# lambdaclass/simpleworks

Hardware: AMD Instinct MI355X
Metric: Marlin prove() constraints/sec at 2^20 R1CS; G1 MSM points/sec (higher is better)
Workload: dtype u32 limbs (384-bit Montgomery Fq for G1, 256-bit Fr); 1 GPU; marlin_prove: synthetic R1CS, 2^20 constraints = variables = non-zeros per matrix (|H| = |K| = 2^20), SRS + proving key device resident; per_gpu_units=1048576, multi_gpu=replicas (one proof per rank)

## Files before the change

simpleworks_amd/_lib.py:

```python
import ctypes
import json
import os

import numpy as np

_HERE = os.path.dirname(os.path.abspath(__file__))
LIB_PATH = os.environ.get("SWM_LIB_PATH") or os.path.join(_HERE, "libswmarlin.so")

_u64p = ctypes.POINTER(ctypes.c_uint64)
_u32p = ctypes.POINTER(ctypes.c_uint32)
_vp = ctypes.c_void_p
_sz = ctypes.c_size_t
_int = ctypes.c_int

ABI = {
    "swm_version": (_int, []),
    "swm_strerror": (ctypes.c_char_p, [_int]),
    "swm_init": (_int, [_int, ctypes.POINTER(_vp)]),
    "swm_destroy": (None, [_vp]),
    "swm_last_error": (ctypes.c_char_p, [_vp]),
    "swm_set_stream": (_int, [_vp, _vp]),
    "swm_set_msm_sharding": (_int, [_vp, ctypes.c_uint, ctypes.c_uint, _vp, _vp]),
    "swm_rccl_unique_id": (_int, [ctypes.c_void_p]),
    "swm_rccl_init": (_int, [_vp, ctypes.c_void_p, ctypes.c_uint, ctypes.c_uint]),
# ... 1225 lines not shown
        self._poly(3, buf, buf.shape[0], 0, z_mont, pc, out)
        return out

    def selftest_ntt_from(self, src_mont, log_n, inverse=False, coset=False):
        src = np.ascontiguousarray(src_mont, dtype=np.uint64).reshape(-1, 4).copy()
        out = np.zeros((1 << log_n, 4), dtype=np.uint64)
        self._poly(4 + int(bool(inverse)) + 2 * int(bool(coset)), src, src.shape[0], log_n, None, None, out)
        return out, src

    def selftest_ntt_cosets(self, coeffs_mont, log_n, ks):
        src = np.ascontiguousarray(coeffs_mont, dtype=np.uint64).reshape(-1, 4).copy()
        kk = np.ascontiguousarray(ks, dtype=np.uint64).reshape(-1)
        out = np.zeros((kk.size << log_n, 4), dtype=np.uint64)
        self._check(self.lib.swm_selftest_poly(self.h, 9, src.ctypes.data, src.shape[0], log_n, _p64(np.zeros(4, np.uint64)),
                                               _p64(kk), kk.size, out.ctypes.data), "swm_selftest_poly")
        return out.reshape(kk.size, 1 << log_n, 4)

    def selftest_intt_cosets3(self, evals_mont, log_n):
        ev = np.ascontiguousarray(evals_mont, dtype=np.uint64).reshape(-1, 4).copy()
        out = np.zeros_like(ev)
        self._poly(10, ev, ev.shape[0], log_n, None, None, out)
        return out

    def selftest_scan(self, words):
        w = np.ascontiguousarray(words, dtype=np.uint32).reshape(-1)
        out = np.zeros(w.size + 1, dtype=np.uint32)
        self._poly(8, w, w.size, 0, None, None, out)
        return out[:-1], int(out[-1])

    def selftest_spmv_plan(self, rowptr, col, val_mont, z_mont):
        rowptr = np.ascontiguousarray(rowptr, dtype=np.uint32)
        col = np.ascontiguousarray(col, dtype=np.uint32)
        val = np.ascontiguousarray(val_mont, dtype=np.uint64).reshape(-1, 4)
        z = np.ascontiguousarray(z_mont, dtype=np.uint64).reshape(-1, 4)
        rows = rowptr.shape[0] - 1
        out = np.zeros((rows, 4), dtype=np.uint64)
        counts = np.zeros(2, dtype=np.uint32)
        self._check(self.lib.swm_selftest_spmv_plan(self.h, _p32(rowptr), _p32(col) if col.size else None,
                                                    _p64(val) if val.size else None, rows, _p64(z), z.shape[0], _p64(out),
                                                    _p32(counts)), "swm_selftest_spmv_plan")
        return out, int(counts[0]), int(counts[1])

    MSM_ROLES = {None: 0, "none": 0, "lead": 1, "follow": 2}
    MSM_DEFER = {"off": 0, "on": 1, "prover": 2}

    def selftest_msm_jobs(self, sets, vectors, jobs, montgomery=False, defer_tail="prover", pipe_min=0):
# ... 23 lines not shown
```

simpleworks_amd/csrc/devops.cuh:

```cuda
#pragma once
#include <chrono>
#include <exception>
#include <functional>
#include <utility>
#include <atomic>
#include "context.h"
#include "ff.cuh"
#include "fill.cuh"
#include "fr29.cuh"
#include "host/chacha.h"
#include "host/marlin_types.h"

namespace swm {

int ntt_run(swm_ctx* ctx, void* d_data, unsigned log_n, int inverse, int coset);
int ntt_run_from(swm_ctx* ctx, void* d_data, unsigned log_n, int inverse, int coset, const void* first_src, size_t src_len);
int ntt_cosets_fwd(swm_ctx* ctx, const void* coeffs, size_t len, unsigned log_n, const unsigned* ks, unsigned ncos, void* out);
int ntt_cosets_inv(swm_ctx* ctx, void* data, unsigned log_n, unsigned ncos);
int ntt_sharded_run(swm_ctx* ctx, void* d_local, unsigned log_n, int inverse, int blocks_in);
struct SpmvPlanHost {
    uint64_t nnz = 0, max_row = 0;
    std::vector<uint32_t> chunks, lrows;
};
struct SpmvPlan {
    uint64_t nnz = 0, max_row = 0;
    const uint32_t* d_chunks = nullptr;
    const uint32_t* d_lrows = nullptr;
    uint32_t n_chunks = 0, n_lrows = 0;
};
void spmv_plan_build(const uint32_t* rowptr, size_t rows, SpmvPlanHost* plan);
int spmv_run(swm_ctx* ctx, const void* d_rowptr, const void* d_col, const void* d_val, const void* d_z, void* d_out,
             size_t rows, const SpmvPlan* plan = nullptr);
int batch_inverse_run(swm_ctx* ctx, void* d, size_t n);

inline void hip_check(swm_ctx* ctx, hipError_t e, const char* what) {
    if (e != hipSuccess) {
        set_err(ctx, SWM_ERR_HIP, "%s: %s", what, hipGetErrorString(e));
        throw MarlinError(e == hipErrorOutOfMemory ? SWM_ERR_OOM : SWM_ERR_HIP, std::string(what) + ": " + hipGetErrorString(e));
    }
}
inline void rc_check(swm_ctx* ctx, int rc) {
    if (rc != SWM_OK) throw MarlinError(rc, ctx->err);
}

template <class T>
struct DBuf {
    swm_ctx* ctx = nullptr;
    T* p = nullptr;
    size_t n = 0, cap = 0;
    DBuf() {}
    DBuf(swm_ctx* c, size_t count) : ctx(c), n(count) {
        void* q = nullptr;
        rc_check(c, pool_alloc(c, (count ? count : 1) * sizeof(T), &q, &cap));
        p = (T*)q;
    }
    DBuf(const DBuf&) = delete;
// ... 824 lines not shown
```

simpleworks_amd/csrc/fr29.cuh:

```cuda
#pragma once
#include "ff.cuh"

namespace swm {

struct Fr29 {
    uint32_t l[9];
};
static constexpr uint32_t M29 = (1u << 29) - 1;
struct Fr29Consts {
    static constexpr uint32_t P[9] = SWM_FR29_P;
    static constexpr uint32_t ONE[9] = SWM_FR29_ONE;
    static constexpr uint32_t P2[9] = SWM_FR29_2P;
};

__device__ __forceinline__ Fr29 fr29_unpack(const Fr& a) {
    Fr29 r;
#pragma unroll
    for (int i = 0; i < 9; i++) {
        const int bit = 29 * i, w = bit >> 5, off = bit & 31;
        uint32_t v = a.v[w] >> off;
        if (off > 3 && w + 1 < 8) v |= a.v[w + 1] << (32 - off);
        r.l[i] = i < 8 ? (v & M29) : v;
    }
    return r;
// ... 17 lines not shown
    return r;
}
__device__ __forceinline__ Fr29 fr29_normalize(const Fr29& a) {
    Fr29 r;
    uint32_t c = 0;
#pragma unroll
    for (int i = 0; i < 8; i++) {
        uint32_t t = a.l[i] + c;
        r.l[i] = t & M29;
        c = t >> 29;
    }
    r.l[8] = a.l[8] + c;
    return r;
}
__device__ __forceinline__ Fr29 fr29_add(const Fr29& a, const Fr29& b) {
    Fr29 r;
#pragma unroll
    for (int i = 0; i < 9; i++) r.l[i] = a.l[i] + b.l[i];
    return r;
}
struct Spread29 {
    uint32_t l[9];
};
__device__ __forceinline__ Fr29 fr29_sub(const Fr29& a, const Fr29& b, const Spread29& sp) {
    Fr29 r;
#pragma unroll
    for (int i = 0; i < 9; i++) r.l[i] = a.l[i] + sp.l[i] - b.l[i];
    return r;
}
__device__ __forceinline__ Fr29 fr29_mul(const Fr29& a, const Fr29& b) {
    Fr29 r;
    uint32_t m[9];
    uint64_t acc = 0;
#pragma unroll
    for (int k = 0; k < 9; k++) {
#pragma unroll
        for (int i = 0; i <= k; i++) acc += (uint64_t)a.l[i] * b.l[k - i];
#pragma unroll
        for (int i = 0; i < k; i++) acc += (uint64_t)m[i] * Fr29Consts::P[k - i];
        m[k] = (0u - (uint32_t)acc) & M29;
        acc = (acc + m[k]) >> 29;
    }
#pragma unroll
    for (int k = 9; k < 17; k++) {
#pragma unroll
        for (int i = k - 8; i < 9; i++) acc += (uint64_t)a.l[i] * b.l[k - i];
// ... 44 lines not shown
```

simpleworks_amd/csrc/marlin.hip:

```cpp
#include <stdlib.h>
#include <string.h>
#include <algorithm>
#include <chrono>
#include <functional>
#include <memory>
#include <type_traits>
#include "devops.cuh"
#include "g1.cuh"
#include "host/ahp.h"

#include "msm.h"
using namespace swm;

#define LAUNCHX(ctx, name, kernel, grid, block, shmem, ...)                         \
    do {                                                                            \
        prof_begin(ctx, name);                                                      \
        hipLaunchKernelGGL(kernel, grid, block, shmem, (ctx)->stream, __VA_ARGS__); \
        prof_end(ctx);                                                              \
        hip_check(ctx, hipGetLastError(), name);                                    \
    } while (0)

#include "host/pk_codec.h"
#include "host/host_handles.h"
struct swm_srs {
    ~swm_srs() {
        if (d_powers) (void)hipFree(d_powers);
    }
    size_t max_degree = 0;
    bool in_subgroup = false;
    G1Affine* d_powers = nullptr;
    std::vector<G1Affine> gamma_powers;
    G2Affine h, beta_h;
};

namespace {

struct DevCsr {
    DBuf<uint32_t> rowptr, col;
    DVec val;
    size_t rows = 0, nnz = 0;
    DBuf<uint32_t> plan_chunks, plan_lrows;
    SpmvPlan plan;
};
struct MatrixArith {
    DVec row, col, val, row_col;
    DVec row_K, col_K, val_K;
    DVec row_B, col_B, val_B, row_col_B;
};
struct GammaTable {
    std::vector<G1Affine> t;
    const G1Affine& at(int j, int w, int d) const { return t[((size_t)j * 64 + w) * 15 + (d - 1)]; }
};

}

struct swm_pk {
    ~swm_pk() {
        if (d_powers) (void)hipFree(d_powers);
        if (d_powers28) (void)hipFree(d_powers28);
        if (d_shifted) (void)hipFree(d_shifted);
        if (d_shifted28) (void)hipFree(d_shifted28);
        if (d_powers_te) (void)hipFree(d_powers_te);
        if (d_shifted_te) (void)hipFree(d_shifted_te);
    }
    int device = 0;
    std::atomic<int> refs{1};
    void own_blocks() {
        for (DevCsr* m : {&a, &b, &c, &at, &bt, &ct}) {
            m->rowptr.detach(); m->col.detach(); m->val.detach(); m->plan_chunks.detach(); m->plan_lrows.detach();
        }
        for (MatrixArith& m : ar)
            for (DVec* v : {&m.row, &m.col, &m.val, &m.row_col, &m.row_K, &m.col_K, &m.val_K, &m.row_B, &m.col_B, &m.val_B, &m.row_col_B})
                v->detach();
    }
    IndexInfo info;
    uint64_t H = 0, K = 0, X = 0, B = 0;
    unsigned logH = 0, logK = 0, logX = 0, logB = 0;
    HostCsr ha, hb, hc;
    DevCsr a, b, c, at, bt, ct;
    MatrixArith ar[3];
    G1Affine* d_powers = nullptr;
    G1Affine* d_powers28 = nullptr;
    G1Affine* d_shifted = nullptr;
    G1Affine* d_shifted28 = nullptr;
    size_t n_powers = 0, n_shifted = 0, shift_base = 0;
    size_t srs_max_degree = 0;
    unsigned tab_c = 0, shtab_c = 0;
    G1TE* d_powers_te = nullptr;
    G1TE* d_shifted_te = nullptr;
    bool in_powers(size_t offset, size_t n) const { return offset + n <= n_powers; }
    void bases_at(size_t offset, size_t n, const G1Affine** b, const G1Affine** b28, MsmTable* tab) const {
        *tab = MsmTable();
        if (in_powers(offset, n)) {
            *b = d_powers + offset;
            *b28 = d_powers28 + offset;
            if (tab_c) *tab = MsmTable{d_powers_te ? nullptr : d_powers28, n_powers, tab_c, offset, d_powers_te};
// ... 617 lines not shown

__device__ __forceinline__ uint64_t reindex_by_subdomain(uint64_t H, uint64_t X, uint64_t index) {
    uint64_t period = H / X;
    if (index < X) return index * period;
    uint64_t i = index - X, x = period - 1;
    return i + (i / x) + 1;
}

void arithmetize(swm_ctx* ctx, swm_pk& pk, const HostCsr& m, MatrixArith& ar) {
    const uint64_t K = pk.K, H = pk.H, X = pk.X;
    std::vector<uint32_t> rows(m.nnz());
    for (size_t r = 0; r < m.rows(); r++)
        for (uint32_t k = m.rowptr[r]; k < m.rowptr[r + 1]; k++) rows[k] = (uint32_t)r;
    DBuf<uint32_t> d_rows(ctx, std::max<size_t>(m.nnz(), 1)), d_cols(ctx, std::max<size_t>(m.nnz(), 1));
    DVec d_vals(ctx, std::max<size_t>(m.nnz(), 1));
    if (m.nnz()) {
        d_rows.upload(rows.data(), m.nnz());
        d_cols.upload(m.col.data(), m.nnz());
        d_vals.upload(m.val.data(), m.nnz());
    }
    ar.row_K = DVec(ctx, K);
    ar.col_K = DVec(ctx, K);
    ar.val_K = DVec(ctx, K);
    DVec rc_K(ctx, K);
    PowTable wt = root_pow_table(ctx, pk.logH);
    Fr h_inv = HDomain(H).size_inv;
    size_t nnz = m.nnz();
    Fr *prow = ar.row_K.p, *pcol = ar.col_K.p, *pval = ar.val_K.p, *prc = rc_K.p;
    const uint32_t *drows = d_rows.p, *dcols = d_cols.p;
    const Fr* dvals = d_vals.p;
    ew(ctx, "index_arith", K, [=] __device__(size_t k) {
        Fr rv, cv, vv;
        if (k < nnz) {
            rv = wt.at(reindex_by_subdomain(H, X, dcols[k]));
            cv = wt.at(drows[k]);
            vv = fp_mul(fp_mul(dvals[k], rv), h_inv);
        } else {
            rv = fp_one<Fr>();
            cv = fp_one<Fr>();
            vv = fp_zero<Fr>();
        }
        prow[k] = rv;
        pcol[k] = cv;
        pval[k] = vv;
        prc[k] = fp_mul(rv, cv);
    });
    auto interp = [&](const DVec& evals) {
        return dv_ntt_from(ctx, evals.p, K, pk.logK, true);
    };
    ar.row = interp(ar.row_K);
    ar.col = interp(ar.col_K);
    ar.val = interp(ar.val_K);
    ar.row_col = interp(rc_K);
    auto on_b = [&](const DVec& coeffs) {
        return dv_ntt_from(ctx, coeffs.p, K, pk.logB, false);
    };
    ar.row_B = on_b(ar.row);
    ar.col_B = on_b(ar.col);
    ar.val_B = on_b(ar.val);
    ar.row_col_B = on_b(ar.row_col);
}

void install_committer_key(swm_ctx* ctx, swm_pk& pk, const G1Affine* powers, size_t n_powers, const G1Affine* shifted,
                           size_t n_shifted, bool device_src, bool in_subgroup) {
// ... 204 lines not shown
        poly[H] = fp_add(poly[H], rho);
    });
}
void div_vh(swm_ctx* ctx, const Fr* q, size_t part, size_t total, Fr* h, Fr* g) {
    ew(ctx, "div_vh", 3 * part, [=] __device__(size_t j) {
        Fr acc = q[j + part];
        if (j + 2 * part < total) acc = fp_add(acc, q[j + 2 * part]);
        if (j + 3 * part < total) acc = fp_add(acc, q[j + 3 * part]);
        h[j] = acc;
        if (j < part) g[j] = fp_add(q[j], acc);
    });
}
void div_vk(swm_ctx* ctx, const Fr* q, size_t part, size_t total, Fr* h) {
    ew(ctx, "div_vk", 3 * part, [=] __device__(size_t j) {
        Fr acc = fp_zero<Fr>();
        for (uint64_t i = 1; j + i * part < total; i++) acc = fp_add(acc, q[j + i * part]);
        h[j] = acc;
    });
}
#ifndef SWM_OUTER_COSETS
#define SWM_OUTER_COSETS 1
#endif
static constexpr uint64_t OUTER_COSETS_MIN_H = 16;
struct Cosets3 {
    Fr p0, p1, p2;
};
__device__ __forceinline__ Cosets3 cosets3_solve(const Fr& u0, const Fr& u1, const Fr& u2, const Fr& iota, const Fr& half) {
    const Fr p1 = fp_mul(fp_sub(u0, u2), half);
    const Fr e = fp_mul(fp_add(u0, u2), half);
    const Fr d = fp_sub(u1, fp_mul(iota, p1));
    return {fp_mul(fp_add(e, d), half), p1, fp_mul(fp_sub(e, d), half)};
}
static Fr fr_half() { return fp_inv(fp_from_u64<Fr>(2)); }
struct RAlphaNumerators {
    Fr n0, n1, n2, n3;
    __device__ __forceinline__ Fr at(size_t i) const {
        const unsigned q = (unsigned)(i & 3);
        return q == 0 ? n0 : q == 1 ? n1 : q == 2 ? n2 : n3;
    }
};
RAlphaNumerators r_alpha_numerators(const Fr& alpha, unsigned logH, uint64_t M) {
    Fr aH = alpha;
    for (unsigned i = 0; i < logH; i++) aH = fp_sqr(aH);
    Fr i4 = HDomain(M).gen;
    for (unsigned i = 0; i < logH; i++) i4 = fp_sqr(i4);
    return {fp_sub(aH, fp_one<Fr>()), fp_sub(aH, i4), fp_sub(aH, fp_sqr(i4)), fp_sub(aH, fp_mul(fp_sqr(i4), i4))};
// ... 19 lines not shown
__device__ __forceinline__ Fr round2_outer_form(const Fr& eta_a, const Fr& eta_b, const Fr& eta_c, const Fr& ra, const Fr& a,
                                                const Fr& b, const Fr& z, const Fr& t) {
    const Fr summed = fp_add(fp_add(fp_mul(eta_c, fp_mul(a, b)), fp_mul(eta_a, a)), fp_mul(eta_b, b));
    return fp_sub(fp_mul(ra, summed), fp_mul(z, t));
}
struct IndexOnB {
    const Fr *ar, *ac, *arc, *av;
    const Fr *br, *bc, *brc, *bv;
    const Fr *cr, *cc, *crc, *cv;
};
struct Round3Challenges {
    Fr alpha, beta, ab, eta_a, eta_b, eta_c, vhab;
};
__device__ __forceinline__ Fr round3_a_minus_bf(const IndexOnB& x, const Round3Challenges& c, size_t i, const Fr& f) {
    Fr da = fp_add(fp_sub(fp_sub(c.ab, fp_mul(x.ar[i], c.alpha)), fp_mul(c.beta, x.ac[i])), x.arc[i]);
    Fr db = fp_add(fp_sub(fp_sub(c.ab, fp_mul(x.br[i], c.alpha)), fp_mul(c.beta, x.bc[i])), x.brc[i]);
    Fr dc = fp_add(fp_sub(fp_sub(c.ab, fp_mul(x.cr[i], c.alpha)), fp_mul(c.beta, x.cc[i])), x.crc[i]);
    Fr dbc = fp_mul(db, dc);
    Fr t = fp_add(fp_add(fp_mul(fp_mul(c.eta_a, x.av[i]), dbc), fp_mul(fp_mul(fp_mul(c.eta_b, x.bv[i]), da), dc)),
                  fp_mul(fp_mul(fp_mul(c.eta_c, x.cv[i]), da), db));
    Fr a_val = fp_mul(c.vhab, t);
    Fr b_val = fp_mul(da, dbc);
    return fp_sub(a_val, fp_mul(b_val, f));
}
struct ProveState {
    ChaChaRng& zk;
    PhaseTrace& tr;
    const ProveShape shape;
    const ShardPlan sp;
    const uint64_t H, K, X, Bsz, M;
    const unsigned logM;
    const size_t nvars, ninst;
    const size_t mask_len;
    const HDomain dh;
    const std::vector<Fr> public_input;
    FiatShamirRng fs;
    VerifierState st;
    Fr rho_w, rho_a, rho_b;
    int lane = 0;
    LPoly P_w, P_za, P_zb, P_mask, P_t, P_g1, P_h1, P_g2, P_h2;
    LPoly idx_polys[12];
    std::map<std::string, LPoly*> polys;
    CommitJob j1[4], j2[3], j3[2];
    std::vector<Commitment> comms1 = std::vector<Commitment>(4), comms2 = std::vector<Commitment>(3),
                            comms3 = std::vector<Commitment>(2);
    bool mask_late = false;
// ... 209 lines not shown
        out[i] = v;
    });
    s.e_z = on_round2_layout(ctx, s, z_poly.p, H + 1);
}

void round1_commitments(swm_ctx* ctx, const swm_pk& pk, ProveState& s) {
    pc_commit_blind(pk, &s.j1[0], &s.zk, &s.P_w.rand);
    pc_commit_blind(pk, &s.j1[1], &s.zk, &s.P_za.rand);
    pc_commit_blind(pk, &s.j1[2], &s.zk, &s.P_zb.rand);
    pc_commit_blind(pk, &s.j1[3], nullptr, &s.P_mask.rand);
    if (s.mask_pieces > 1) {
        Fr c0 = s.mask.download(0, 1)[0];
        Fr c0s = fp_to_std(c0);
        G1XYZZ extra = g1_mul_limbs(pk.vk.vk.g, c0s.v, 8);
        for (unsigned k = 0; k + 1 < s.mask_pieces; k++) g1_add(extra, commit_wait(ctx, &s.mask_part[k]));
        s.j1[3].has_extra = true;
        s.j1[3].extra = extra;
    }
    commit_gather(ctx, {&s.j1[0].plain, &s.j1[1].plain, &s.j1[2].plain, &s.j1[3].plain});
    pc_commit_end_round(ctx, pk, {&s.j1[0], &s.j1[1], &s.j1[2], &s.j1[3]}, {&s.zk, &s.zk, &s.zk, nullptr},
                        {&s.P_w.rand, &s.P_za.rand, &s.P_zb.rand, &s.P_mask.rand}, s.comms1.data());
}

void r_alpha_on_h(swm_ctx* ctx, const swm_pk& pk, ProveState& s) {
    const Fr alpha = s.st.alpha;
    PowTable wh = root_pow_table(ctx, pk.logH);
    Fr* rh = s.r_alpha_evals.p;
    ew(ctx, "r_alpha_den", s.H, [=] __device__(size_t i) { rh[i] = fp_sub(alpha, wh.at(i)); });
    rc_check(ctx, batch_inverse_run(ctx, rh, s.H));
    Fr vh = s.dh.vanishing(alpha);
    ew(ctx, "r_alpha_scale", s.H, [=] __device__(size_t i) { rh[i] = fp_mul(rh[i], vh); });
}
void r_alpha(swm_ctx* ctx, const swm_pk& pk, ProveState& s) {
    const Fr alpha = s.st.alpha;
    s.r_alpha_evals = DVec(ctx, s.H);
    {
        Fr a4h = alpha;
        for (unsigned i = 0; i < s.logM; i++) a4h = fp_sqr(a4h);
        s.ra_closed_form = !fp_is_one(a4h) && !sw(SW_RALPHA_TRANSFORMS);
    }
    if (!s.ra_closed_form) return r_alpha_on_h(ctx, pk, s);
    const size_t n = s.cosets ? 3 * s.H : s.sp.Mloc;
    s.e_ra = DVec(ctx, n);
    PowTable wt = root_pow_table(ctx, s.logM);
    Fr* out = s.e_ra.p;
    Fr* rh = s.r_alpha_evals.p;
    const RAlphaNumerators nu = r_alpha_numerators(alpha, pk.logH, s.M);
    with_product_map(s.sp, s.sp.r2, n, s.cosets, pk.logH, [&](auto map) {
        ew(ctx, "r_alpha_den", n, [=] __device__(size_t p) { out[p] = fp_sub(alpha, wt.at(map.index(p))); });
        rc_check(ctx, batch_inverse_run(ctx, out, n));
        ew(ctx, "r_alpha_scale", n, [=] __device__(size_t p) {
            const size_t i = map.index(p);
            const Fr v = fp_mul(out[p], nu.at(i));
            out[p] = v;
            if constexpr (!std::is_same_v<decltype(map), BlocksMap>)
                if ((i & 3) == 0) rh[i >> 2] = v;
        });
    });
// ... 28 lines not shown
                if (k % ratio != 0) {
                    const size_t wi = k - k / ratio - 1;
                    zk = wi < nwit ? zz[ninst + wi] : fp_zero<Fr>();
                }
                q[k] = round2_outer_form(eta_a, eta_b, eta_c, rh[k], za[k], zb[k], zk, th[k]);
            });
        }
        dv_ntt(ctx, s.t_poly, pk.logH, true);
    }
    s.tr.tick("r2: t polynomial enqueued");
    s.P_t.p = s.t_poly.p;
    s.P_t.n = H;
    pc_commit_begin(ctx, pk, &s.lane, s.P_t.p, s.P_t.n, false, 0, false, &s.j2[0]);
}

void round2_q1(swm_ctx* ctx, const swm_pk& pk, ProveState& s) {
    const uint64_t H = s.H, M = s.M;
    const size_t Mloc = s.sp.Mloc;
    const Fr eta_a = s.st.eta_a, eta_b = s.st.eta_b, eta_c = s.st.eta_c;
    const size_t off = s.cosets ? H : 0, n = s.cosets ? 2 * H : Mloc;
    if (!s.cosets) s.q1 = DVec(ctx, Mloc);
    const Fr* mp = s.mask.p;
    {
        const Fr* pra = s.e_ra.p + off;
        if (!s.ra_closed_form) {
            DVec ra_poly = dv_ntt_from(ctx, s.r_alpha_evals.p, H, pk.logH, true);
            s.e_ra = on_round2_layout(ctx, s, ra_poly.p, H);
            pra = s.e_ra.p;
        }
        DVec e_t = on_round2_layout(ctx, s, s.t_poly.p, H);
        Fr* out = s.q1.p + off;
        const Fr *pza = s.e_za.p, *pzb = s.e_zb.p, *pt = e_t.p, *pz = s.e_z.p;
        ew(ctx, "round2_pointwise", n, [=] __device__(size_t i) {
            out[i] = round2_outer_form(eta_a, eta_b, eta_c, pra[i], pza[i], pzb[i], pz[i], pt[i]);
        });
        s.e_za.release();
        s.e_zb.release();
        s.e_z.release();
    }
    s.h1 = DVec(ctx, 3 * H);
    s.g1x = DVec(ctx, H);
    Fr* q = s.q1.p;
    if (s.cosets) {
        rc_check(ctx, ntt_cosets_inv(ctx, q, pk.logH, 3));
        Fr *h = s.h1.p, *g = s.g1x.p;
        const Fr iota = HDomain(4).gen, half = fr_half();
        ew(ctx, "q1_cosets_solve_div_vh", H, [=] __device__(size_t j) {
            const Cosets3 c = cosets3_solve(q[j], q[j + H], q[j + 2 * H], iota, half);
            const Fr p0 = fp_add(c.p0, mp[j]), p1 = fp_add(c.p1, mp[j + H]), p2 = fp_add(c.p2, mp[j + 2 * H]);
            const Fr hj = fp_add(p1, p2);
            h[j] = hj;
// ... 35 lines not shown
    pc_commit_begin(ctx, pk, &s.lane, s.P_h1.p, s.P_h1.n, false, 0, false, &s.j2[2]);
    pc_commit_begin(ctx, pk, &s.lane, s.P_g1.p, s.P_g1.n, true, H - 2, true, &s.j2[1]);
    commit_flush(ctx);
    Fr rem0 = s.g1x.download(0, 1)[0];
    bool unsat = !fp_is_zero(rem0);
    pc_commit_blind(pk, &s.j2[0], nullptr, &s.P_t.rand);
    pc_commit_blind(pk, &s.j2[1], &s.zk, &s.P_g1.rand);
    pc_commit_blind(pk, &s.j2[2], nullptr, &s.P_h1.rand);
    commit_gather(ctx, {&s.j2[0].plain, &s.j2[1].plain, &s.j2[1].shifted, &s.j2[2].plain});
    pc_commit_end_round(ctx, pk, {&s.j2[0], &s.j2[1], &s.j2[2]}, {nullptr, &s.zk, nullptr},
                        {&s.P_t.rand, &s.P_g1.rand, &s.P_h1.rand}, s.comms2.data());
    if (unsat && !ctx->emulated_exchange)
        throw MarlinError(SWM_ERR_UNSATISFIED, "outer sumcheck does not hold: constraint system is not satisfied");
}

void round3_polys(swm_ctx* ctx, const swm_pk& pk, ProveState& s) {
    const uint64_t K = s.K, Bsz = s.Bsz;
    const Fr alpha = s.st.alpha, beta = s.st.beta;
    const Fr eta_a = s.st.eta_a, eta_b = s.st.eta_b, eta_c = s.st.eta_c;
    const Fr vhab = fp_mul(s.dh.vanishing(alpha), s.dh.vanishing(beta));
    s.f = DVec(ctx, K);
    const bool f_cosets = SWM_OUTER_COSETS && !s.sp.r3 && Bsz == 4 * K && K >= OUTER_COSETS_MIN_H;
    DVec f_K;
    {
        DVec inv(ctx, 3 * K);
        for (int m = 0; m < 3; m++) {
            Fr* out = inv.p + (size_t)m * K;
            const Fr *rk = pk.ar[m].row_K.p, *ck = pk.ar[m].col_K.p;
            ew(ctx, "round3_den_K", K, [=] __device__(size_t i) { out[i] = fp_mul(fp_sub(beta, rk[i]), fp_sub(alpha, ck[i])); });
        }
        rc_check(ctx, batch_inverse_run(ctx, inv.p, 3 * K));
        Fr* out = s.f.p;
        const Fr *ia = inv.p, *ib = inv.p + K, *ic = inv.p + 2 * K;
        const Fr *va = pk.ar[0].val_K.p, *vb = pk.ar[1].val_K.p, *vc = pk.ar[2].val_K.p;
        if (f_cosets) {
            f_K = DVec(ctx, K);
            out = f_K.p;
        }
        ew(ctx, "round3_f_K", K, [=] __device__(size_t i) {
            Fr t = fp_add(fp_add(fp_mul(fp_mul(eta_a, va[i]), ia[i]), fp_mul(fp_mul(eta_b, vb[i]), ib[i])),
                          fp_mul(fp_mul(eta_c, vc[i]), ic[i]));
            out[i] = fp_mul(vhab, t);
        });
        if (f_cosets) rc_check(ctx, ntt_run_from(ctx, s.f.p, pk.logK, 1, 0, f_K.p, K));
        else dv_ntt(ctx, s.f, pk.logK, true);
    }
    s.P_g2.p = s.f.p + 1; s.P_g2.n = K - 1; s.P_g2.has_bound = true; s.P_g2.bound = K - 2;
// ... 838 lines not shown
}
int swm_pk_deserialize(swm_ctx* ctx, const uint8_t* bytes, size_t len, swm_pk** out) {
    return swm_pk_deserialize_ex(ctx, bytes, len, 0, out);
}
int swm_r1cs_is_satisfied(swm_ctx* ctx, const swm_r1cs* cs, int* ok, size_t* first_bad) {
    if (!ctx || !cs || !ok) return SWM_ERR_INVALID_ARG;
    SWM_ON_DEVICE(ctx);
    SWM_GUARD(ctx, is_satisfied_impl(ctx, cs, ok, first_bad));
}

static void selftest_poly_impl(swm_ctx* ctx, int op, void* data, size_t n, size_t m, const uint64_t* z, const uint64_t* pieces,
                               size_t npieces, void* out) {
    Fr zz = fp_zero<Fr>();
    if (z) memcpy(zz.v, z, 32);
    if (op == 8) {
        DBuf<uint32_t> in(ctx, n), res(ctx, n);
        if (n) in.upload((const uint32_t*)data, n);
        const uint32_t total = scan_exclusive_u32(ctx, in.p, res.p, n);
        std::vector<uint32_t> h = res.download(0, n);
        if (n) memcpy(out, h.data(), n * 4);
        ((uint32_t*)out)[n] = total;
        return;
    }
    DVec a(ctx, n);
    if (n) a.upload((const Fr*)data, n);
    if (op == 9) {
        unsigned ks[4];
        for (size_t c = 0; c < npieces; c++) ks[c] = (unsigned)pieces[c];
        DVec t(ctx, npieces << m);
        rc_check(ctx, ntt_cosets_fwd(ctx, a.p, n, (unsigned)m, ks, (unsigned)npieces, t.p));
        std::vector<Fr> h = t.download(0, t.n);
        memcpy(out, h.data(), t.n * sizeof(Fr));
        return;
    }
    if (op == 10) {
        const size_t N = (size_t)1 << m;
        rc_check(ctx, ntt_cosets_inv(ctx, a.p, (unsigned)m, 3));
        DVec t(ctx, 3 * N);
        const Fr* u = a.p;
        Fr* o = t.p;
        const Fr iota = HDomain(4).gen, half = fr_half();
        ew(ctx, "cosets3_solve", N, [=] __device__(size_t j) {
            const Cosets3 c = cosets3_solve(u[j], u[j + N], u[j + 2 * N], iota, half);
            o[j] = c.p0;
            o[j + N] = c.p1;
            o[j + 2 * N] = c.p2;
// ... 13 lines not shown
    } else if (op == 2) {
        const Fr v = poly_eval(ctx, a.p, n, zz);
        memcpy(out, v.v, sizeof(Fr));
    } else if (op == 3) {
        for (size_t i = 0; i < npieces; i++)
            if (pieces[2 * i] > n || pieces[2 * i + 1] > n - pieces[2 * i]) throw MarlinError(SWM_ERR_INVALID_ARG, "piece out of range");
        DVec res(ctx, npieces);
        std::vector<EvalItem> items;
        for (size_t i = 0; i < npieces; i++) items.push_back({a.p + pieces[2 * i], (size_t)pieces[2 * i + 1], res.p + i});
        EvalPoint ep = eval_point(ctx, zz);
        poly_eval_many(ctx, items, ep);
        std::vector<Fr> h = res.download(0, npieces);
        if (npieces) memcpy(out, h.data(), npieces * sizeof(Fr));
    } else {
        DVec t = dv_ntt_from(ctx, a.p, n, (unsigned)m, ((op - 4) & 1) != 0, ((op - 4) & 2) != 0);
        std::vector<Fr> h = t.download(0, t.n);
        memcpy(out, h.data(), t.n * sizeof(Fr));
        std::vector<Fr> s = a.download(0, n);
        if (n) memcpy(data, s.data(), n * sizeof(Fr));
    }
}
int swm_selftest_poly(swm_ctx* ctx, int op, void* data, size_t n, size_t m, const uint64_t z[4], const uint64_t* pieces,
                      size_t npieces, void* out) {
    if (!ctx || op < 0 || op > 10 || (n && !data)) return SWM_ERR_INVALID_ARG;
    if ((op >= 1 && op <= 3 && !z) || (op == 0 && (!z || m == 0)) || (op != 0 && !out) || (op == 3 && npieces && !pieces))
        return SWM_ERR_INVALID_ARG;
    if (op >= 4 && op <= 7 && (m < 1 || m > 28 || n > ((size_t)1 << m))) return SWM_ERR_INVALID_ARG;
    if (op == 9) {
        if (m < 1 || m > 26 || n > ((size_t)2 << m) || npieces < 1 || npieces > 4 || !pieces) return SWM_ERR_INVALID_ARG;
        for (size_t c = 0; c < npieces; c++)
            if (pieces[c] > 3) return SWM_ERR_INVALID_ARG;
    }
    if (op == 10 && (m < 1 || m > 26 || n != ((size_t)3 << m))) return SWM_ERR_INVALID_ARG;
    SWM_ON_DEVICE(ctx);
    SWM_GUARD(ctx, selftest_poly_impl(ctx, op, data, n, m, z, pieces, npieces, out));
}
static void selftest_spmv_plan_impl(swm_ctx* ctx, const uint32_t* rowptr, const uint32_t* col, const uint64_t* val, size_t rows,
                                    const uint64_t* z, size_t z_len, uint64_t* out, uint32_t* plan_counts) {
    const size_t nnz = rowptr[rows];
    HostCsr m;
    m.rowptr.assign(rowptr, rowptr + rows + 1);
    m.col.assign(col, col + nnz);
    m.val.resize(nnz);
    if (nnz) memcpy(m.val.data(), val, nnz * sizeof(Fr));
    DevCsr d = upload_csr(ctx, m);
    DVec dz(ctx, z_len), o(ctx, rows);
    dz.upload((const Fr*)z, z_len);
// ... 103 lines not shown
```

simpleworks_amd/csrc/ntt.hip:

```cpp
#include <atomic>
#include "context.h"
#include "ff.cuh"
#include "fr29.cuh"
#include <string.h>
#include <algorithm>
#include <vector>

namespace swm {

static constexpr int NTT_THREADS = 256;
static constexpr unsigned NTT_MAX_LOG_R = 10;

struct NttPassArgs {
    const Fr* src;
    Fr* dst;
    unsigned log_n, log_r, log_ns;
    const Fr* tw_small;
    const Fr* tw_lo;
    const Fr* tw_hi;
    const Fr* cs_lo;
    const Fr* cs_hi;
    uint64_t src_len;
    const Fr* pass_tw;
    int coset_in;
// ... 354 lines not shown
    static const bool off = sw(SW_NTT_PASS_TABLES) == 0;
    if (off) return SWM_OK;
    const uint64_t key = (1ull << 51) | ((uint64_t)log_n << 20) | ((uint64_t)log_ns << 10) | ((uint64_t)log_r << 1) | (inverse ? 1 : 0);
    auto it = ctx->ntt_small.find(key);
    if (it == ctx->ntt_small.end()) {
        const size_t count = (size_t)1 << (log_ns + log_r);
        if (ctx->ntt_pass_table_bytes + count * sizeof(Fr) > ((size_t)4 << 30)) return SWM_OK;
        void* d = nullptr;
        if (hipMalloc(&d, count * sizeof(Fr)) != hipSuccess) {
            (void)hipGetLastError();
            return SWM_OK;
        }
        hipLaunchKernelGGL(ntt_build_pass_tw, dim3((unsigned)((count + 255) / 256)), dim3(256), 0, ctx->stream,
                           reinterpret_cast<const Fr*>(rt29->lo), reinterpret_cast<const Fr*>(rt29->hi), log_ns, log_r,
                           log_n - log_ns - log_r, reinterpret_cast<Fr*>(d));
        SWM_HIP(ctx, hipGetLastError());
        ctx->ntt_pass_table_bytes += count * sizeof(Fr);
        it = ctx->ntt_small.emplace(key, d).first;
    }
    *out = reinterpret_cast<const Fr*>(it->second);
    return SWM_OK;
}

static Spread29 lazy_spread(unsigned k, unsigned borrows) {
    Spread29 sp;
    uint64_t carry = 0;
    for (int i = 0; i < 9; i++) {
        uint64_t t = (uint64_t)Fr29Consts::P[i] * k + carry;
        sp.l[i] = i < 8 ? (uint32_t)(t & M29) : (uint32_t)t;
        carry = t >> 29;
    }
    sp.l[0] += borrows << 29;
    for (int i = 1; i < 8; i++) sp.l[i] += (borrows << 29) - borrows;
    sp.l[8] -= borrows;
    return sp;
}
static LazyPlan lazy_plan(unsigned log_r, unsigned b_in) {
    LazyPlan P;
    memset(&P, 0, sizeof(P));
    unsigned B = b_in;
    P.r2 = lazy_spread(2 * B, 1);
    if (log_r & 1) B = std::max(2 * B, 2u);
    const unsigned nsteps = log_r / 2;
    for (unsigned st = 0; st < nsteps && st < 6; st++) {
        P.s1[st] = lazy_spread(2 * B, 1);
        P.s2[st] = lazy_spread(4 * B, 2);
        const bool red = 4 * B > 64 || st + 1 == nsteps;
        if (red) P.reduce |= 1u << st;
        B = red ? 4 : 4 * B;
    }
    P.s4 = lazy_spread(4, 1);
    P.out_below_2r = B <= 2 ? 1u : 0u;
    return P;
}

int ntt_run_from(swm_ctx* ctx, void* d_data, unsigned log_n, int inverse, int coset, const void* first_src, size_t src_len);
int ntt_run(swm_ctx* ctx, void* d_data, unsigned log_n, int inverse, int coset) {
    return ntt_run_from(ctx, d_data, log_n, inverse, coset, nullptr, 0);
}
// ... 220 lines not shown
```

simpleworks_amd/csrc/vec.hip:

```cpp
#include <string.h>
#include "context.h"
#include "fq28.cuh"
#include "fr29.cuh"
#include "frinv.cuh"
#include "g1.cuh"

namespace swm {

__global__ void __launch_bounds__(256) vec_mul_kernel(const Fr* __restrict__ a, const Fr* __restrict__ b,
                                                      Fr* __restrict__ out, size_t n) {
    SWM_LIGHT_KERNEL();
    for (size_t i = blockIdx.x * (size_t)blockDim.x + threadIdx.x; i < n; i += (size_t)gridDim.x * blockDim.x)
        out[i] = fp_mul(a[i], b[i]);
}

static constexpr int BINV_CHUNK = 16, BINV_CHUNK_SMALL = 4;
static constexpr int BINV_THREADS = 256;
template <int BINV_CHUNK>
__global__ void __launch_bounds__(BINV_THREADS) batch_inverse_kernel29(Fr* __restrict__ v, size_t n) {
    SWM_LIGHT_KERNEL();
    __shared__ Fr sp[BINV_THREADS], ss[BINV_THREADS];
    __shared__ Fr s_inv;
    const unsigned tid = threadIdx.x;
    size_t t = blockIdx.x * (size_t)blockDim.x + tid;
// ... 37 lines not shown
            }
        }
    }
}

int vec_mul_run(swm_ctx* ctx, const void* a, const void* b, void* out, size_t n) {
    if (n == 0) return SWM_OK;
    unsigned grid = (unsigned)std::min<size_t>((n + 255) / 256, 256 * 32);
    SWM_LAUNCH(ctx, "vec_mul", vec_mul_kernel, dim3(grid), dim3(256), 0, (const Fr*)a, (const Fr*)b, (Fr*)out, n);
    return SWM_OK;
}
int batch_inverse_run(swm_ctx* ctx, void* d, size_t n) {
    if (n == 0) return SWM_OK;
    static constexpr size_t small_below = 262144;
    if (n <= small_below) {
        const size_t threads = (n + BINV_CHUNK_SMALL - 1) / BINV_CHUNK_SMALL;
        const dim3 grid((unsigned)((threads + BINV_THREADS - 1) / BINV_THREADS));
        SWM_LAUNCH(ctx, "batch_inverse", batch_inverse_kernel29<BINV_CHUNK_SMALL>, grid, dim3(BINV_THREADS), 0, (Fr*)d, n);
        return SWM_OK;
    }
    const size_t threads = (n + BINV_CHUNK - 1) / BINV_CHUNK;
    const dim3 grid((unsigned)((threads + BINV_THREADS - 1) / BINV_THREADS));
    SWM_LAUNCH(ctx, "batch_inverse", batch_inverse_kernel29<BINV_CHUNK>, grid, dim3(BINV_THREADS), 0, (Fr*)d, n);
    return SWM_OK;
}

template <class F>
__global__ void __launch_bounds__(256) selftest_mul_kernel(const F* a, const F* b, F* out, size_t n) {
    size_t i = blockIdx.x * (size_t)blockDim.x + threadIdx.x;
    if (i < n) out[i] = fp_mul(a[i], b[i]);
}
template <class F>
__global__ void __launch_bounds__(256) selftest_mul_chain(F* out, int iters) {
    size_t i = blockIdx.x * (size_t)blockDim.x + threadIdx.x;
    F a = fp_one<F>(), b = fp_one<F>();
    a.v[0] ^= (uint32_t)i;
    b.v[1] ^= (uint32_t)(i * 2654435761u);
    for (int k = 0; k < iters; k++) {
        a = fp_mul(a, b);
        b = fp_mul(b, a);
    }
    out[i] = fp_add(a, b);
}
__global__ void __launch_bounds__(256) selftest_mul28_kernel(const Fq* a, const Fq* b, Fq* out, size_t n) {
    size_t i = blockIdx.x * (size_t)blockDim.x + threadIdx.x;
    if (i < n) out[i] = fq28_pack(fq28_canonical(fq28_mul(fq28_unpack(a[i]), fq28_unpack(b[i]))));
// ... 160 lines not shown
```

Before: 22.74 million constraints/s.

## Compute Lagrange-kernel evaluations via product tower and gather-based round-3 f

Replaces the batch-inverse computation of r(alpha, X) on H (and on the round-2 cosets) with a multiplicative product-tower kernel that builds the evaluations from squared powers of the challenge. Round 3 no longer inverts per-matrix denominators over K. Instead it evaluates r(beta, .) on H with the same tower and gathers r_beta[row] * r_alpha[col] using new uint32 index arrays stored in the proving key. This trades batch inversions and some NTT work for random-access gathers and extra key memory, and adds selftests for the new kernels.

Result: no change. 22.90 million constraints/s (median of 6 runs) (+0.7%).

```diff
diff --git a/simpleworks_amd/_lib.py b/simpleworks_amd/_lib.py
--- a/simpleworks_amd/_lib.py
+++ b/simpleworks_amd/_lib.py
@@ -1271,6 +1271,39 @@
         self._poly(10, ev, ev.shape[0], log_n, None, None, out)
         return out
 
+    R_TOWER_LAYOUTS = {"pieces": 0, "dense": 1, "h": 2}
+
+    def selftest_r_tower(self, c_mont, log_n, cosets, layout="pieces"):
+        kk = np.ascontiguousarray(cosets, dtype=np.uint64).reshape(-1)
+        n = 1 << log_n
+        rows = {"pieces": kk.size * n, "dense": 4 * n, "h": n}[layout]
+        out = np.zeros((rows, 4), dtype=np.uint64)
+        zz = np.ascontiguousarray(c_mont, dtype=np.uint64).reshape(4)
+        self._check(self.lib.swm_selftest_poly(self.h, 11, None, self.R_TOWER_LAYOUTS[layout], log_n, _p64(zz), _p64(kk), kk.size,
+                                               out.ctypes.data), "swm_selftest_poly")
+        return out.reshape(kk.size, n, 4) if layout == "pieces" else out
+
+    def selftest_round3_f(self, r_beta_mont, r_alpha_mont, vals_mont, idx, etas_mont):
+        rb = np.ascontiguousarray(r_beta_mont, dtype=np.uint64).reshape(-1, 4)
+        ra = np.ascontiguousarray(r_alpha_mont, dtype=np.uint64).reshape(-1, 4)
+        ix = np.ascontiguousarray(idx, dtype=np.uint32)
+        K = ix.shape[-1]
+        va = np.ascontiguousarray(vals_mont, dtype=np.uint64).reshape(3 * K, 4)
+        assert ra.shape == rb.shape and ix.shape == (3, 2, K)
+        data = np.ascontiguousarray(np.concatenate([rb, ra, va, np.asarray(etas_mont, dtype=np.uint64).reshape(3, 4)]))
+        words = np.zeros((6 * K + 1) // 2, dtype=np.uint64)
+        words.view(np.uint32)[:6 * K] = ix.reshape(-1)
+        out = np.zeros((K, 4), dtype=np.uint64)
+        self._check(self.lib.swm_selftest_poly(self.h, 12, data.ctypes.data, rb.shape[0], K, _p64(np.zeros(4, np.uint64)),
+                                               _p64(words), words.size, out.ctypes.data), "swm_selftest_poly")
+        return out
+
+    def selftest_pk_index_arrays(self, pk_handle, K):
+        out = np.zeros((3, 2, K), dtype=np.uint32)
+        self._check(self.lib.swm_selftest_poly(self.h, 13, pk_handle, K, 0, _p64(np.zeros(4, np.uint64)), None, 0,
+                                               out.ctypes.data), "swm_selftest_poly")
+        return out
+
     def selftest_scan(self, words):
         w = np.ascontiguousarray(words, dtype=np.uint32).reshape(-1)
         out = np.zeros(w.size + 1, dtype=np.uint32)
diff --git a/simpleworks_amd/csrc/devops.cuh b/simpleworks_amd/csrc/devops.cuh
--- a/simpleworks_amd/csrc/devops.cuh
+++ b/simpleworks_amd/csrc/devops.cuh
@@ -32,6 +32,7 @@
 int spmv_run(swm_ctx* ctx, const void* d_rowptr, const void* d_col, const void* d_val, const void* d_z, void* d_out,
              size_t rows, const SpmvPlan* plan = nullptr);
 int batch_inverse_run(swm_ctx* ctx, void* d, size_t n);
+int r_tower_run(swm_ctx* ctx, const void* c, unsigned m, const unsigned* cosets, unsigned ncos, int dense, void* out);
 
 inline void hip_check(swm_ctx* ctx, hipError_t e, const char* what) {
     if (e != hipSuccess) {
diff --git a/simpleworks_amd/csrc/fr29.cuh b/simpleworks_amd/csrc/fr29.cuh
--- a/simpleworks_amd/csrc/fr29.cuh
+++ b/simpleworks_amd/csrc/fr29.cuh
@@ -63,6 +63,19 @@
 struct Spread29 {
     uint32_t l[9];
 };
+inline Spread29 lazy_spread(unsigned k, unsigned borrows) {
+    Spread29 sp;
+    uint64_t carry = 0;
+    for (int i = 0; i < 9; i++) {
+        uint64_t t = (uint64_t)Fr29Consts::P[i] * k + carry;
+        sp.l[i] = i < 8 ? (uint32_t)(t & M29) : (uint32_t)t;
+        carry = t >> 29;
+    }
+    sp.l[0] += borrows << 29;
+    for (int i = 1; i < 8; i++) sp.l[i] += (borrows << 29) - borrows;
+    sp.l[8] -= borrows;
+    return sp;
+}
 __device__ __forceinline__ Fr29 fr29_sub(const Fr29& a, const Fr29& b, const Spread29& sp) {
     Fr29 r;
 #pragma unroll
diff --git a/simpleworks_amd/csrc/marlin.hip b/simpleworks_amd/csrc/marlin.hip
--- a/simpleworks_amd/csrc/marlin.hip
+++ b/simpleworks_amd/csrc/marlin.hip
@@ -46,6 +46,7 @@
     DVec row, col, val, row_col;
     DVec row_K, col_K, val_K;
     DVec row_B, col_B, val_B, row_col_B;
+    DBuf<uint32_t> row_idx, col_idx;
 };
 struct GammaTable {
     std::vector<G1Affine> t;
@@ -72,6 +73,10 @@
         for (MatrixArith& m : ar)
             for (DVec* v : {&m.row, &m.col, &m.val, &m.row_col, &m.row_K, &m.col_K, &m.val_K, &m.row_B, &m.col_B, &m.val_B, &m.row_col_B})
                 v->detach();
+        for (MatrixArith& m : ar) {
+            m.row_idx.detach();
+            m.col_idx.detach();
+        }
     }
     IndexInfo info;
     uint64_t H = 0, K = 0, X = 0, B = 0;
@@ -735,6 +740,8 @@
     ar.row_K = DVec(ctx, K);
     ar.col_K = DVec(ctx, K);
     ar.val_K = DVec(ctx, K);
+    ar.row_idx = DBuf<uint32_t>(ctx, K);
+    ar.col_idx = DBuf<uint32_t>(ctx, K);
     DVec rc_K(ctx, K);
     PowTable wt = root_pow_table(ctx, pk.logH);
     Fr h_inv = HDomain(H).size_inv;
@@ -742,17 +749,23 @@
     Fr *prow = ar.row_K.p, *pcol = ar.col_K.p, *pval = ar.val_K.p, *prc = rc_K.p;
     const uint32_t *drows = d_rows.p, *dcols = d_cols.p;
     const Fr* dvals = d_vals.p;
+    uint32_t *pri = ar.row_idx.p, *pci = ar.col_idx.p;
     ew(ctx, "index_arith", K, [=] __device__(size_t k) {
         Fr rv, cv, vv;
+        uint32_t ri = 0, ci = 0;
         if (k < nnz) {
-            rv = wt.at(reindex_by_subdomain(H, X, dcols[k]));
-            cv = wt.at(drows[k]);
+            ri = (uint32_t)reindex_by_subdomain(H, X, dcols[k]);
+            ci = drows[k];
+            rv = wt.at(ri);
+            cv = wt.at(ci);
             vv = fp_mul(fp_mul(dvals[k], rv), h_inv);
         } else {
             rv = fp_one<Fr>();
             cv = fp_one<Fr>();
             vv = fp_zero<Fr>();
         }
+        pri[k] = ri;
+        pci[k] = ci;
         prow[k] = rv;
         pcol[k] = cv;
         pval[k] = vv;
@@ -1003,6 +1016,9 @@
 #define SWM_OUTER_COSETS 1
 #endif
 static constexpr uint64_t OUTER_COSETS_MIN_H = 16;
+#ifndef SWM_PRELUDE_PRODUCTS
+#define SWM_PRELUDE_PRODUCTS 1
+#endif
 struct Cosets3 {
     Fr p0, p1, p2;
 };
@@ -1068,6 +1084,21 @@
     Fr a_val = fp_mul(c.vhab, t);
     Fr b_val = fp_mul(da, dbc);
     return fp_sub(a_val, fp_mul(b_val, f));
+}
+struct Round3Tables {
+    Fr eta[3];
+    const Fr* val[3];
+    const uint32_t *row_idx[3], *col_idx[3];
+};
+void round3_f_on_k(swm_ctx* ctx, const Fr* r_beta, const Fr* r_alpha, const Round3Tables& tables, size_t K, Fr* out) {
+    const Round3Tables x = tables;
+    ew(ctx, "round3_f_K", K, [=] __device__(size_t k) {
+        Fr acc = fp_zero<Fr>();
+#pragma unroll
+        for (int m = 0; m < 3; m++)
+            acc = fp_add(acc, fp_mul(fp_mul(x.eta[m], x.val[m][k]), fp_mul(r_beta[x.row_idx[m][k]], r_alpha[x.col_idx[m][k]])));
+        out[k] = acc;
+    });
 }
 struct ProveState {
     ChaChaRng& zk;
@@ -1323,18 +1354,33 @@
                         {&s.P_w.rand, &s.P_za.rand, &s.P_zb.rand, &s.P_mask.rand}, s.comms1.data());
 }
 
+void r_on_h(swm_ctx* ctx, const swm_pk& pk, const Fr& c, Fr* out) {
+    static const unsigned h_alone[1] = {0};
+    rc_check(ctx, r_tower_run(ctx, &c, pk.logH, h_alone, 1, 0, out));
+}
 void r_alpha_on_h(swm_ctx* ctx, const swm_pk& pk, ProveState& s) {
     const Fr alpha = s.st.alpha;
+    Fr* rh = s.r_alpha_evals.p;
+    if (SWM_PRELUDE_PRODUCTS) return r_on_h(ctx, pk, alpha, rh);
     PowTable wh = root_pow_table(ctx, pk.logH);
-    Fr* rh = s.r_alpha_evals.p;
     ew(ctx, "r_alpha_den", s.H, [=] __device__(size_t i) { rh[i] = fp_sub(alpha, wh.at(i)); });
     rc_check(ctx, batch_inverse_run(ctx, rh, s.H));
     Fr vh = s.dh.vanishing(alpha);
     ew(ctx, "r_alpha_scale", s.H, [=] __device__(size_t i) { rh[i] = fp_mul(rh[i], vh); });
 }
+void r_alpha_rest(swm_ctx* ctx, const swm_pk& pk, ProveState& s) {
+    static const unsigned rest[2] = {1, 2}, all[4] = {0, 1, 2, 3};
+    s.e_ra = DVec(ctx, s.cosets ? 2 * s.H : s.M);
+    if (s.cosets) rc_check(ctx, r_tower_run(ctx, &s.st.alpha, pk.logH, rest, 2, 0, s.e_ra.p));
+    else rc_check(ctx, r_tower_run(ctx, &s.st.alpha, pk.logH, all, 4, 1, s.e_ra.p));
+}
 void r_alpha(swm_ctx* ctx, const swm_pk& pk, ProveState& s) {
     const Fr alpha = s.st.alpha;
     s.r_alpha_evals = DVec(ctx, s.H);
+    if (SWM_PRELUDE_PRODUCTS && !s.sp.r2) {
+        s.ra_closed_form = !sw(SW_RALPHA_TRANSFORMS);
+        return r_alpha_on_h(ctx, pk, s);
+    }
     {
         Fr a4h = alpha;
         for (unsigned i = 0; i < s.logM; i++) a4h = fp_sqr(a4h);
@@ -1409,11 +1455,16 @@
     if (!s.cosets) s.q1 = DVec(ctx, Mloc);
     const Fr* mp = s.mask.p;
     {
-        const Fr* pra = s.e_ra.p + off;
+        const Fr* pra;
         if (!s.ra_closed_form) {
             DVec ra_poly = dv_ntt_from(ctx, s.r_alpha_evals.p, H, pk.logH, true);
             s.e_ra = on_round2_layout(ctx, s, ra_poly.p, H);
             pra = s.e_ra.p;
+        } else if (SWM_PRELUDE_PRODUCTS && !s.sp.r2) {
+            r_alpha_rest(ctx, pk, s);
+            pra = s.e_ra.p;
+        } else {
+            pra = s.e_ra.p + off;
         }
         DVec e_t = on_round2_layout(ctx, s, s.t_poly.p, H);
         Fr* out = s.q1.p + off;
@@ -1495,7 +1546,24 @@
     s.f = DVec(ctx, K);
     const bool f_cosets = SWM_OUTER_COSETS && !s.sp.r3 && Bsz == 4 * K && K >= OUTER_COSETS_MIN_H;
     DVec f_K;
-    {
+    if (SWM_PRELUDE_PRODUCTS) {
+        DVec r_beta(ctx, s.H);
+        r_on_h(ctx, pk, beta, r_beta.p);
+        Fr* out = s.f.p;
+        if (f_cosets) {
+            f_K = DVec(ctx, K);
+            out = f_K.p;
+        }
+        Round3Tables t{{eta_a, eta_b, eta_c}, {}, {}, {}};
+        for (int m = 0; m < 3; m++) {
+            t.val[m] = pk.ar[m].val_K.p;
+            t.row_idx[m] = pk.ar[m].row_idx.p;
+            t.col_idx[m] = pk.ar[m].col_idx.p;
+        }
+        round3_f_on_k(ctx, r_beta.p, s.r_alpha_evals.p, t, K, out);
+        if (f_cosets) rc_check(ctx, ntt_run_from(ctx, s.f.p, pk.logK, 1, 0, f_K.p, K));
+        else dv_ntt(ctx, s.f, pk.logK, true);
+    } else {
         DVec inv(ctx, 3 * K);
         for (int m = 0; m < 3; m++) {
             Fr* out = inv.p + (size_t)m * K;
@@ -2380,6 +2448,47 @@
         ((uint32_t*)out)[n] = total;
         return;
     }
+    if (op == 11) {
+        unsigned ks[4];
+        for (size_t c = 0; c < npieces; c++) ks[c] = (unsigned)pieces[c];
+        DVec t = dv_zeros(ctx, (n == 1 ? 4 : npieces) << m);
+        rc_check(ctx, r_tower_run(ctx, &zz, (unsigned)m, ks, (unsigned)npieces, n == 1, t.p));
+        std::vector<Fr> h = t.download(0, t.n);
+        memcpy(out, h.data(), t.n * sizeof(Fr));
+        return;
+    }
+    if (op == 12) {
+        const size_t H = n, K = m;
+        const uint32_t* idx = (const uint32_t*)pieces;
+        for (size_t i = 0; i < 6 * K; i++)
+            if (idx[i] >= H) throw MarlinError(SWM_ERR_INVALID_ARG, "index outside H");
+        DVec a(ctx, 2 * H + 3 * K + 3), f(ctx, K);
+        a.upload((const Fr*)data, a.n);
+        DBuf<uint32_t> di(ctx, 6 * K);
+        di.upload(idx, 6 * K);
+        const Fr* eta = (const Fr*)data + 2 * H + 3 * K;
+        Round3Tables t{{eta[0], eta[1], eta[2]}, {}, {}, {}};
+        for (int j = 0; j < 3; j++) {
+            t.val[j] = a.p + 2 * H + j * K;
+            t.row_idx[j] = di.p + 2 * j * K;
+            t.col_idx[j] = di.p + (2 * j + 1) * K;
+        }
+        round3_f_on_k(ctx, a.p, a.p + H, t, K, f.p);
+        std::vector<Fr> h = f.download(0, K);
+        memcpy(out, h.data(), K * sizeof(Fr));
+        return;
+    }
+    if (op == 13) {
+        const swm_pk& pk = *(const swm_pk*)data;
+        if (n != pk.K || pk.device != ctx->device) throw MarlinError(SWM_ERR_INVALID_ARG, "not this key's |K|, or not its device");
+        for (int j = 0; j < 3; j++) {
+            const uint32_t* src[2] = {pk.ar[j].row_idx.p, pk.ar[j].col_idx.p};
+            for (int k = 0; k < 2; k++)
+                hip_check(ctx, hipMemcpyAsync((uint32_t*)out + (2 * j + k) * n, src[k], n * 4, hipMemcpyDeviceToHost, ctx->stream), "d2h");
+        }
+        hip_check(ctx, hipStreamSynchronize(ctx->stream), "sync");
+        return;
+    }
     DVec a(ctx, n);
     if (n) a.upload((const Fr*)data, n);
     if (op == 9) {
@@ -2439,7 +2548,16 @@
 }
 int swm_selftest_poly(swm_ctx* ctx, int op, void* data, size_t n, size_t m, const uint64_t z[4], const uint64_t* pieces,
                       size_t npieces, void* out) {
-    if (!ctx || op < 0 || op > 10 || (n && !data)) return SWM_ERR_INVALID_ARG;
+    if (!ctx || op < 0 || op > 13 || (n && !data && op != 11)) return SWM_ERR_INVALID_ARG;
+    if (op == 11) {
+        if (m > 24 || n > 2 || !z || npieces < 1 || npieces > 4 || !pieces || (n == 2 && (npieces != 1 || pieces[0] != 0)))
+            return SWM_ERR_INVALID_ARG;
+        for (size_t c = 0; c < npieces; c++)
+            if (pieces[c] > 3) return SWM_ERR_INVALID_ARG;
+    }
+    if (op == 12 && (n < 1 || m < 1 || n > ((size_t)1 << 28) || m > ((size_t)1 << 28) || !pieces || npieces < (6 * m + 1) / 2))
+        return SWM_ERR_INVALID_ARG;
+    if (op == 13 && (!data || n < 1)) return SWM_ERR_INVALID_ARG;
     if ((op >= 1 && op <= 3 && !z) || (op == 0 && (!z || m == 0)) || (op != 0 && !out) || (op == 3 && npieces && !pieces))
         return SWM_ERR_INVALID_ARG;
     if (op >= 4 && op <= 7 && (m < 1 || m > 28 || n > ((size_t)1 << m))) return SWM_ERR_INVALID_ARG;
diff --git a/simpleworks_amd/csrc/ntt.hip b/simpleworks_amd/csrc/ntt.hip
--- a/simpleworks_amd/csrc/ntt.hip
+++ b/simpleworks_amd/csrc/ntt.hip
@@ -400,19 +400,6 @@
     return SWM_OK;
 }
 
-static Spread29 lazy_spread(unsigned k, unsigned borrows) {
-    Spread29 sp;
-    uint64_t carry = 0;
-    for (int i = 0; i < 9; i++) {
-        uint64_t t = (uint64_t)Fr29Consts::P[i] * k + carry;
-        sp.l[i] = i < 8 ? (uint32_t)(t & M29) : (uint32_t)t;
-        carry = t >> 29;
-    }
-    sp.l[0] += borrows << 29;
-    for (int i = 1; i < 8; i++) sp.l[i] += (borrows << 29) - borrows;
-    sp.l[8] -= borrows;
-    return sp;
-}
 static LazyPlan lazy_plan(unsigned log_r, unsigned b_in) {
     LazyPlan P;
     memset(&P, 0, sizeof(P));
diff --git a/simpleworks_amd/csrc/vec.hip b/simpleworks_amd/csrc/vec.hip
--- a/simpleworks_amd/csrc/vec.hip
+++ b/simpleworks_amd/csrc/vec.hip
@@ -83,6 +83,105 @@
     const size_t threads = (n + BINV_CHUNK - 1) / BINV_CHUNK;
     const dim3 grid((unsigned)((threads + BINV_THREADS - 1) / BINV_THREADS));
     SWM_LAUNCH(ctx, "batch_inverse", batch_inverse_kernel29<BINV_CHUNK>, grid, dim3(BINV_THREADS), 0, (Fr*)d, n);
+    return SWM_OK;
+}
+
+static constexpr unsigned TOWER_MAX_LOG = 28;
+static constexpr unsigned TOWER_DIRECT_MAX = 8;
+static constexpr unsigned TOWER_R = 3;
+struct TowerArgs {
+    Fr csq[TOWER_MAX_LOG];
+    Fr init;
+    Spread29 sp2;
+    const Fr *lo, *hi;
+    Fr* out;
+    unsigned m, top, direct, first, ncos, jshift;
+    unsigned cosets[4];
+    size_t piece;
+};
+__device__ __forceinline__ Fr29 tower_twiddle(const TowerArgs& a, uint64_t e) {
+    return fr29_mul_fenced(fr29_unpack(a.lo[e & 1023]), fr29_unpack(a.hi[e >> 10]));
+}
+template <int R>
+__global__ void __launch_bounds__(256) r_tower_kernel(TowerArgs a) {
+    SWM_LIGHT_KERNEL();
+    const unsigned log_top = a.m - a.top;
+    const size_t t = blockIdx.x * (size_t)blockDim.x + threadIdx.x;
+    if (t >= ((size_t)a.ncos << log_top)) return;
+    const unsigned ci = (unsigned)(t >> log_top);
+    const uint64_t i = t & (((uint64_t)1 << log_top) - 1);
+    const uint64_t k = a.cosets[ci];
+    Fr* out = a.out + (a.piece ? ci * a.piece : (size_t)k);
+    Fr29 v[1 << R];
+    if (a.first) {
+        Fr29 acc = fr29_unpack(a.init);
+        for (unsigned l = a.top + a.direct; l-- > a.top;) {
+            const uint64_t j = i & (((uint64_t)1 << (a.m - l)) - 1);
+            acc = fr29_mul_fenced(fr29_add(fr29_unpack(a.csq[l]), tower_twiddle(a, (k + 4 * j) << l)), acc);
+        }
+        v[0] = acc;
+    } else {
+        v[0] = fr29_unpack(out[i << a.jshift]);
+    }
+#pragma unroll
+    for (int r = 0; r < R; r++) {
+        const unsigned l = a.top - 1 - r;
+        const Fr29 c = fr29_unpack(a.csq[l]);
+#pragma unroll
+        for (int u = 0; u < (1 << r); u++) {
+            const uint64_t j = i + ((uint64_t)u << log_top);
+            const Fr29 x = tower_twiddle(a, (k + 4 * j) << l), p = v[u];
+            v[u] = fr29_mul_fenced(fr29_add(c, x), p);
+            v[u + (1 << r)] = fr29_mul_fenced(fr29_sub(c, x, a.sp2), p);
+        }
+    }
+#pragma unroll
+    for (int u = 0; u < (1 << R); u++)
+        out[(i + ((uint64_t)u << log_top)) << a.jshift] = fr29_pack(fr29_canonical(v[u], true));
+}
+int r_tower_run(swm_ctx* ctx, const void* c, unsigned m, const unsigned* cosets, unsigned ncos, int dense, void* out) {
+    if (m > TOWER_MAX_LOG || ncos < 1 || ncos > 4) return set_err(ctx, SWM_ERR_INVALID_ARG, "r_tower: bad shape");
+    unsigned seen = 0;
+    for (unsigned i = 0; i < ncos; i++) {
+        if (cosets[i] > 3 || (seen >> cosets[i] & 1)) return set_err(ctx, SWM_ERR_INVALID_ARG, "r_tower: bad coset list");
+        seen |= 1u << cosets[i];
+    }
+    NttTables* wt = nullptr;
+    SWM_TRY(get_root_tables(ctx, m + 2, 0, &wt));
+    TowerArgs a;
+    memset(&a, 0, sizeof(a));
+    static const Fr lambda = fp_inv(fp_from_u64<Fr>(32)), lambda_inv2 = fp_from_u64<Fr>(1024);
+    Fr cl = *(const Fr*)c;
+    a.init = fp_one<Fr>();
+    for (unsigned l = 0; l < m; l++) {
+        a.csq[l] = fp_mul(cl, lambda);
+        cl = fp_sqr(cl);
+        a.init = fp_mul(a.init, lambda_inv2);
+    }
+    a.sp2 = lazy_spread(2, 1);
+    a.lo = (const Fr*)wt->lo;
+    a.hi = (const Fr*)wt->hi;
+    a.out = (Fr*)out;
+    a.m = m;
+    a.ncos = ncos;
+    for (unsigned i = 0; i < ncos; i++) a.cosets[i] = cosets[i];
+    a.jshift = dense ? 2 : 0;
+    a.piece = dense ? 0 : (size_t)1 << m;
+    a.direct = m <= TOWER_DIRECT_MAX ? m : TOWER_DIRECT_MAX - 2 + m % TOWER_R;
+    a.first = 1;
+    a.top = m - a.direct;
+    do {
+        const size_t lanes = (size_t)ncos << (m - a.top);
+        const dim3 grid((unsigned)((lanes + 255) / 256));
+        if (a.top) {
+            SWM_LAUNCH(ctx, "r_tower", r_tower_kernel<TOWER_R>, grid, dim3(256), 0, a);
+            a.top -= TOWER_R;
+        } else {
+            SWM_LAUNCH(ctx, "r_tower", r_tower_kernel<0>, grid, dim3(256), 0, a);
+        }
+        a.first = 0;
+        a.direct = 0;
+    } while (a.top);
     return SWM_OK;
 }
 
```
